# Equim-chan/Mortal

Measured on AMD Instinct MI355X. Metric: env steps/sec (65536 parallel tables per GPU), higher is better.
Workload: dtype u8/i32 state, f32 obs

## Files before the change

### mortal_amd/csrc/mj_capi.hip

```cpp
#include <hip/hip_runtime.h>

#include <algorithm>
#include <cmath>
#include <cstdio>
#include <cstring>
#include <optional>
#include <string>
#include <vector>

#include "../../include/mortal_amd.h"
#include "mj_step.hip"
#include "mj_replay.hip"
#include "mj_encode.hip"
#include "mj_sp.hip"

static_assert(sizeof(MjAlgoQuery) == 72, "MjAlgoQuery layout");
__global__ __launch_bounds__(64) void mj_k_algo_query(const MjAlgoQuery* q, int n, MjAlgoResult* out) {
    const int i = blockIdx.x * 64 + threadIdx.x;
    if (i >= n) return;
    const MjAlgoQuery Q = q[i];
    MjAlgoResult R = {0, 0, 0, 0, 0, 0, 0, 0};
    Hand h = {0, 0};
    for (int t = 0; t < 34; t++)
        for (int c = 0; c < (int)Q.tehai[t] && c < 4; c++) h.inc(t);
// ... 975 lines not shown
                    sp_[8], sp_[0], sp_[1], sp_[2], sp_[3], sp_[4], sp_[9], sp_[5], sp_[10], sp_[7]);
            for (int k = 11; k < 32; k++) fprintf(stderr, " %llu", sp_[k]);
            fprintf(stderr, "\n");
        }
    }
#endif
    if (!P) return fail("null pool");
    HIP_OK(hipStreamSynchronize((hipStream_t)stream));
    unsigned long long tmp[8];
    HIP_OK(hipMemcpy(tmp, P->counters, sizeof tmp, hipMemcpyDeviceToHost));
    for (int i = 0; i < 8; i++) out[i] = tmp[i];
    out[5] = P->cycles;
    int f = 0;
    HIP_OK(hipMemcpy(&f, P->enc_flag, sizeof f, hipMemcpyDeviceToHost));
    out[6] = (unsigned long long)f;
    if (P->sp.err) {
        unsigned long long e2[SP_ERR_WORDS];
        HIP_OK(hipMemcpy(e2, P->sp.err, sizeof e2, hipMemcpyDeviceToHost));
        out[6] += e2[SP_ERR_OVERFLOW];
        out[7] = e2[SP_ERR_ROWS];
        const unsigned long long* pass = e2 + SP_ERR_PASS;
        if (P->knobs.sp_prof)
            fprintf(stderr, "[sp prof] rows %llu setup %llu expand %llu evalL0 %llu evalL>0 %llu encode %llu states %llu (wall_clock64 ticks, 100 MHz) | "
                    "expand passes: probes %llu lists+V %llu td-probes %llu layout %llu inserts %llu; items %llu expanded %llu edges %llu l0-entries %llu; level-0 probe %llu scoring %llu; workgroup lifetimes: sum %llu max %llu queue pops %llu hash resets %llu; eval wavefront time %llu; shader clock %.0f MHz (s_memtime cycles %llu over the lifetimes)\n",
                    e2[SP_ERR_ROWS], e2[SP_ERR_T_SETUP], e2[SP_ERR_T_EXPAND], e2[SP_ERR_T_EVAL0], e2[SP_ERR_T_EVAL], e2[SP_ERR_T_WRITE], e2[SP_ERR_STATES],
                    pass[0], pass[1], pass[2], pass[3], pass[4], pass[5], pass[6], e2[SP_ERR_EDGES], e2[SP_ERR_L0_ITEMS],
                    e2[SP_ERR_T_L0_PROBE], e2[SP_ERR_T_L0_SCORE], e2[SP_ERR_WG_LIFE], e2[SP_ERR_WG_LIFE_MAX], e2[SP_ERR_T_POP], e2[SP_ERR_T_RESET],
                    e2[SP_ERR_T_EVAL_WAVE], e2[SP_ERR_WG_LIFE] ? 100.0 * (double)e2[SP_ERR_WG_CLOCK] / (double)e2[SP_ERR_WG_LIFE] : 0.0,
                    e2[SP_ERR_WG_CLOCK]);
    }
    return 0;
}

int mj_sp_phase_ticks(MjPool* P, uint64_t out[8], void* stream) {
    if (!P) return fail("null pool");
    for (int i = 0; i < 8; i++) out[i] = 0;
    if (!P->sp.err) return 0;
    HIP_OK(hipStreamSynchronize((hipStream_t)stream));
    unsigned long long e2[8];
    HIP_OK(hipMemcpy(e2, P->sp.err, sizeof e2, hipMemcpyDeviceToHost));
    for (int i = 0; i < 8; i++) out[i] = e2[i];
    return 0;
}

int mj_pool_set_sp_schedule(MjPool* P, int mode, int max_rows, int wide_grid, int min_level1, int min_level2) {
    if (!P) return fail("null pool");
    if (P->sp.work && mode != 0 && mode >= -1 && P->sp.spare == 0) return fail("mj_pool_set_sp_schedule: the work areas are allocated (call it before the first obs-v4 mj_encode)");
    if (mode >= -1) P->sp_wide_mode = mode > 0 ? 1 : mode;
    if (max_rows > 0) P->sp_wide_max_rows = max_rows;
    if (wide_grid > 0) P->sp_wide_grid = std::min(wide_grid, 256);
    if (min_level1 > 0) P->sp_promo_min[1] = min_level1;
    if (min_level2 > 0) P->sp_promo_min[2] = min_level2;
    P->sp_sched_set = true;
    return 0;
}

int mj_sp_schedule_stats(MjPool* P, uint64_t out[4], void* stream) {
    if (!P) return fail("null pool");
    for (int i = 0; i < 4; i++) out[i] = 0;
    if (!P->sp.err) return 0;
    HIP_OK(hipStreamSynchronize((hipStream_t)stream));
    unsigned long long e2[SP_ERR_WORDS];
    HIP_OK(hipMemcpy(e2, P->sp.err, sizeof e2, hipMemcpyDeviceToHost));
    out[0] = P->sp_hybrid_launches;
    out[1] = e2[SP_ERR_PROMOTED];
    out[2] = e2[SP_ERR_SWEPT];
// ... 47 lines not shown
```

### mortal_amd/csrc/mj_sp.hip

```cpp
#include <hip/hip_runtime.h>

#include <type_traits>

#include "mj_rules.h"
#include "mj_sptab.h"


#ifndef SP_THREADS
#define SP_THREADS 256
#endif
#define SP_CAP 16384
#define SP_T 17
#define SP_MAX_CAND 14
#ifndef SP_NS
#define SP_NS 16
#endif
#ifndef SP_SORT_MIN
#define SP_SORT_MIN 8
#endif
#ifndef SP_ITEM_CAP
#define SP_ITEM_CAP 64
#endif
#ifndef SP_WPS
#define SP_WPS 4
#endif
#define SP_WGS (4 * SP_WPS * 64 / SP_THREADS)

#ifndef SP_CC_N
#define SP_CC_N 2048
#endif
#ifndef SP_TAIL_BATCH
#define SP_TAIL_BATCH 4
#endif
#define SP_Q_TAIL 32
#define SP_Q_PROMO_DONE 96
#define SP_PROMO_LEVELS 2
#define SP_Q_PROMO_ALLOC(p) (128 + 64 * (p))
#define SP_Q_PROMO_HEAD(p) (160 + 64 * (p))
#define SP_Q_PROMO_ENT 256
#ifndef SP_PROMO_CAP
#define SP_PROMO_CAP 512
#endif
#define SP_Q_WORDS (SP_Q_PROMO_ENT + SP_PROMO_CAP)
#ifndef SP_WIDE_THREADS
#define SP_WIDE_THREADS 1024
#endif
#define SP_POOL (SP_CAP * 32)
#define SP_ITEMS (SP_CAP * 4)
#define SP_L0_MAX 17
#define SP_EL_SLOT(v) ((v) & (SP_CAP - 1))
#define SP_EL_IDX(v) ((v) >> 14)
struct alignas(128) SpNode {
    float val[SP_T][3];
    u8 pad_[52];
};
static_assert(sizeof(SpNode) == 256 && offsetof(SpNode, val) == 0, "SpNode layout");
struct alignas(16) SpHdr {
    u32 child_off;
    unsigned short n_ch;
    u8 sumreq, n_ent;
    u64 l0cnt2;
};
static_assert(sizeof(SpHdr) == 16 && offsetof(SpHdr, n_ch) == 4 && offsetof(SpHdr, sumreq) == 6 && offsetof(SpHdr, l0cnt2) == 8,
              "the evaluation reads the header as one or two u64");
struct SpKeys {
    u64 k0, k1, k2, k3;
    u64 dk;
};
#define SP_ENT_SLOT(e) ((e) & 0x3FFFu)
#define SP_ENT_KEY(e) (((e) >> 14) & 511u)
#define SP_ENT_LAST (1u << 23)
#define SP_ENT_COUNT(e) (((e) >> 24) & 7u)
#define SP_ENT_INVALID (1u << 27)
struct alignas(16) SpF4 { float x, y, z, w; };
#define SP_HANDOFF_WORDS 1024
struct alignas(128) SpWork {
    u64 tag[SP_CAP];
    SpNode node[SP_CAP];
    SpKeys keys[SP_CAP];
    SpHdr hdr[SP_CAP];
    u32 list[SP_CAP];
    u32 elist[SP_CAP];
    u32 pool[SP_POOL];
    u32 items[SP_ITEMS];
    SpF4 l0sc[SP_ITEMS];
    u32 epoch;
    u32 pad_[31];
    alignas(16) u32 handoff[SP_HANDOFF_WORDS];
#ifdef MJ_EMU
    u32 idx_of[SP_CAP];
#endif
};
static_assert(offsetof(SpWork, node) % 128 == 0 && sizeof(SpWork) % 128 == 0, "nodes on line boundaries");

#define SP_NT_ROWS 124
#define SP_NT_STRIDE (SP_T + 3)
__constant__ const float* c_sp_nt;
static inline void sp_not_tsumo_build(float* out ) {
    for (int n_left = 0; n_left < SP_NT_ROWS; n_left++)
        for (int q = 0; q < SP_NT_ROWS; q++) {
            float* r = out + ((size_t)n_left * SP_NT_ROWS + q) * SP_NT_STRIDE;
            const bool row_on = q <= 122 && q < n_left + 1;
            const int lim = n_left - q;
            float cur = row_on ? 1.f : 0.f;
            for (int j = 0; j < SP_NT_STRIDE; j++) r[j] = 0.f;
            r[0] = cur;
            for (int j = 0; j < SP_T - 1; j++) {
                cur = (row_on && j < lim) ? cur * (float)(n_left - q - j) / (float)(n_left - j) : 0.f;
                r[j + 1] = cur;
            }
        }
}

struct SpParams {
    const TableOne* snap;
    const uint32_t* rows;
    int n_rows;
    MjTablesDev tables;
    float* obs;
    SpWork* work;
    int* queue;
    const uint32_t* order;
    unsigned long long* prof;
// ... 68 lines not shown
};
MJD void sp_discard(SpState& s, int tile) {
    s.h.dec(deaka(tile));
    if (is_aka(tile)) s.akas &= ~(1u << (tile - T_5MR));
}
MJD void sp_deal(SpState& s, int tile) {
    s.w.dec(deaka(tile));
    s.h.inc(deaka(tile));
    if (is_aka(tile)) {
        s.akas &= ~(8u << (tile - T_5MR));
        s.akas |= 1u << (tile - T_5MR);
    }
}
MJD void sp_key(const SpState& s, u64 k[4]) {
    k[0] = s.h.mp;
    k[1] = s.h.sz | ((u64)(s.akas & 7) << 48);
    k[2] = s.w.mp;
    k[3] = s.w.sz | ((u64)((s.akas >> 3) & 7) << 48);
}

struct alignas(16) SpCtx {
    Melds melds;
    int len_div3, bakaze, jikaze, is_menzen, num_doras_in_fuuro, n_dora, calc_double_riichi, calc_haitei,
        prefer_riichi, T, n_left;
    int dora_ind[5];
    float tsumo_prob[4][SP_T];
    int lvl_begin[5], lvl_end[5];
    int n_list;
    int n_pool;
    int n_items;
    int overflow;
    unsigned long long* prof;
    unsigned long long pt[8];
    unsigned long long* cc;
    unsigned cc_epoch;
    unsigned tag_epoch;
    int n_cand;
    int cand_tile[SP_MAX_CAND], cand_slot[SP_MAX_CAND], cand_down[SP_MAX_CAND], cand_nreq[SP_MAX_CAND];
    u64 cand_req[SP_MAX_CAND];
    u64 spec_req[2][34];
    u64 row7x[2];
    signed char colcand[36];
    int order[SP_MAX_CAND];
    float cand_tp0[SP_MAX_CAND], cand_wp0[SP_MAX_CAND], cand_ev0[SP_MAX_CAND];
};

#if defined(__HIP_DEVICE_COMPILE__)
#define SP_ASSUME_LDS(p) __builtin_assume(__builtin_amdgcn_is_shared((const void*)(p)))
#else
#define SP_ASSUME_LDS(p) ((void)0)
#endif
#ifdef MJ_EMU
#define SP_HBM
#else
#define SP_HBM __attribute__((address_space(1)))
#endif

#if defined(__HIP_DEVICE_COMPILE__) && !defined(MJ_EMU)
template <class Tp> __device__ __forceinline__ Tp* sp_uniform(Tp* p) {
    const unsigned long long v = (unsigned long long)p;
    const unsigned lo = __builtin_amdgcn_readfirstlane((unsigned)v), hi = __builtin_amdgcn_readfirstlane((unsigned)(v >> 32));
    return (Tp*)(((unsigned long long)hi << 32) | lo);
}
#else
template <class Tp> MJD Tp* sp_uniform(Tp* p) { return p; }
#endif
template <class Tv, class Bp> __device__ __forceinline__ Tv sp_ld(Bp base, u32 byte_off) {
// ... 28 lines not shown
#ifdef MJ_EMU
    *reinterpret_cast<SpF3*>(reinterpret_cast<char*>(base) + byte_off) = SpF3{x, y, z};
#else
    SP_HBM SpF3* p = reinterpret_cast<SP_HBM SpF3*>(reinterpret_cast<SP_HBM char*>(base) + (unsigned long long)byte_off);
    p->x = x; p->y = y; p->z = z;
#endif
}
MJD int sp_f2i(float v) {
#if defined(MJ_EMU)
    return v != v ? 0 : v >= 2147483648.f ? 2147483647 : v <= -2147483648.f ? (-2147483647 - 1) : (int)v;
#else
    return (int)v;
#endif
}

MJD u64 sp_dk_add(u64 dk, int draw_tile, int discard_tile) {
    u32 d0 = (u32)dk & 63, d1 = (u32)(dk >> 6) & 63, d2 = (u32)(dk >> 12) & 63;
    u32 x0 = (u32)(dk >> 18) & 63, x1 = (u32)(dk >> 24) & 63, x2 = (u32)(dk >> 30) & 63, x3 = (u32)(dk >> 36) & 63;
    if (draw_tile >= 0) {
        u32 x = (u32)draw_tile + 1, t;
        t = max(d0, x); x = min(d0, x); d0 = t;
        t = max(d1, x); x = min(d1, x); d1 = t;
        d2 = max(d2, x);
    }
    if (discard_tile >= 0) {
        u32 x = (u32)discard_tile + 1, t;
        t = max(x0, x); x = min(x0, x); x0 = t;
        t = max(x1, x); x = min(x1, x); x1 = t;
        t = max(x2, x); x = min(x2, x); x2 = t;
        x3 = max(x3, x);
    }
    return (u64)(d0 | (d1 << 6) | (d2 << 12) | (x0 << 18) | (x1 << 24)) | ((u64)(x2 | (x3 << 6)) << 30);
}
MJD u32 sp_dk_pos(u64 dk) {
    u32 h = (u32)dk * 0x9E3779B1u ^ ((u32)(dk >> 32) + 0x7F4A7C15u) * 0x85EBCA77u;
    h ^= h >> 15;
    return (h * 0x2C1B3C6Du) >> 18;
}
static_assert(SP_CAP == 1 << 14, "sp_dk_pos returns 14 bits");
#define SP_EPOCH_MAX 0x1FFFFFu
#ifndef SP_EPOCH_WRAP
#define SP_EPOCH_WRAP SP_EPOCH_MAX
#endif
#define SP_TAG(dk, ep) ((dk) | ((u64)(ep) << 42) | (1ull << 63))
MJD bool sp_tag_free(u64 t, u32 ep) { return (u32)((t >> 42) & SP_EPOCH_MAX) != ep; }

#ifndef SP_OPAQUE_TID
#define SP_OPAQUE_TID 2
#endif
#if defined(MJ_EMU)
#define SP_OPQ(level, v) (v)
#else
__device__ __forceinline__ int sp_opaque_v(int v) { asm volatile("" : "+v"(v)); return v; }
#define SP_OPQ(level, v) ((SP_OPAQUE_TID) >= (level) ? sp_opaque_v(v) : (v))
#endif
#if defined(MJ_EMU) || !defined(SP_OPAQUE_PTR)
#define SP_OPQ_PTR(level, p) (p)
#else
template <typename Tp> __device__ __forceinline__ Tp* sp_opaque_s(Tp* p) { asm volatile("" : "+s"(p)); return p; }
#define SP_OPQ_PTR(level, p) ((SP_OPAQUE_PTR) >= (level) ? sp_opaque_s(p) : (p))
#endif
#ifndef SP_ATTR_EXPAND
#define SP_ATTR_EXPAND __forceinline__
#endif
#ifndef SP_ATTR_L0P
#define SP_ATTR_L0P __noinline__
#endif
#ifndef SP_ATTR_L0S
#define SP_ATTR_L0S __noinline__
#endif
#ifndef SP_ATTR_EVAL
#define SP_ATTR_EVAL __noinline__
// ... 1 lines not shown
#ifndef SP_ATTR_EVAL0
#define SP_ATTR_EVAL0 __noinline__
#endif

template <class TagP>
MJD u64 sp_claim_tag(TagP tagp, u64 h, u64 seen) {
    u64 expected = seen;
    __hip_atomic_compare_exchange_strong(tagp, &expected, h, __ATOMIC_RELAXED, __ATOMIC_RELAXED, __HIP_MEMORY_SCOPE_AGENT);
    return expected == seen ? 0ull : expected;
}
MJD SpState sp_apply(SpState s, int tile, int dt) {
    if (tile >= 0) sp_deal(s, tile);
    if (dt >= 0) sp_discard(s, dt);
    return s;
}
template <class WP>
__device__ __forceinline__ void sp_new_state(WP W, SpCtx* X, u32 slot, u64 dk, const SpState& st) {
    const int idx = atomicAdd(&X->n_list, 1);
    if (idx < SP_CAP) {
        u64 k[4];
        sp_key(st, k);
        W->list[idx] = slot;
        auto& e = W->keys[idx];
        e.k0 = k[0]; e.k1 = k[1]; e.k2 = k[2]; e.k3 = k[3]; e.dk = dk;
#ifdef MJ_EMU
        W->idx_of[slot] = (u32)idx;
#endif
    } else {
        X->overflow = 1;
    }
}
#ifdef MJ_EMU
template <class WP>
inline void sp_emu_check_hit(WP W, SpCtx* X, u32 slot, const SpState& st) {
    u64 k[4];
    sp_key(st, k);
    const auto& e = W->keys[W->idx_of[slot]];
    if (e.k0 != k[0] || e.k1 != k[1] || e.k2 != k[2] || e.k3 != k[3]) X->overflow = 1;
}
#endif
template <class WP>
__device__ __forceinline__ int sp_insert(WP W, SpCtx* X, u64 dk, const SpState& base, int tile, int dt) {
    const u32 ep = X->tag_epoch;
    const u64 tag = SP_TAG(dk, ep);
    u32 pos = sp_dk_pos(dk);
    for (int probe = 0; probe < SP_CAP; probe++) {
        u64 old = W->tag[pos];
        if (sp_tag_free(old, ep)) old = sp_claim_tag(&W->tag[pos], tag, old);
        if (old == 0ull) {
            sp_new_state(W, X, pos, dk, sp_apply(base, tile, dt));
            return (int)pos;
        }
        if (old == tag) {
#ifdef MJ_EMU
            sp_emu_check_hit(W, X, pos, sp_apply(base, tile, dt));
#endif
            return (int)pos;
        }
        pos = (pos + 1) & (SP_CAP - 1);
    }
    X->overflow = 1;
    return -1;
}
template <class NodeT>
MJD SpState sp_state_of(const NodeT& n) {
    SpState s;
    s.h.mp = n.k0;
    s.h.sz = n.k1 & 0xFFFFFFFFFFFFull;
    s.w.mp = n.k2;
    s.w.sz = n.k3 & 0xFFFFFFFFFFFFull;
    s.akas = (u32)((n.k1 >> 48) & 7) | ((u32)((n.k3 >> 48) & 7) << 3);
    return s;
}

__device__ bool sp_get_score(const MjTablesDev& T, const SpCtx* X, const SpState& s, int win_tile, float scores[4]) {
    AgariIn in;
    in.tehai = s.h;
    {
        const Melds& xm = X->melds;
        in.m.chis = xm.chis; in.m.pons = xm.pons; in.m.minkans = xm.minkans; in.m.ankans = xm.ankans;
        in.m.n_chis = xm.n_chis; in.m.n_pons = xm.n_pons; in.m.n_minkans = xm.n_minkans; in.m.n_ankans = xm.n_ankans;
    }
    in.is_menzen = X->is_menzen != 0;
    in.bakaze = X->bakaze;
    in.jikaze = X->jikaze;
    in.winning_tile = deaka(win_tile);
    in.is_ron = false;
    const bool is_oya = X->jikaze == T_E;
    const int additional = X->is_menzen ? (X->prefer_riichi ? 2 : 1) : 0;
    int num_doras = 0;
// ... 248 lines not shown
            const bool aka = sp_aka_in_wall(S, t);
            cnt += (!aka || S.w.get(t) >= 2) + aka;
            sumreq += S.w.get(t);
        }
        u64 cnt2 = 0;
        if (cnt > SP_L0_MAX) { X->overflow = 1; cnt = SP_L0_MAX; }
        const int base = atomicAdd(&X->n_items, cnt);
        int e = 0;
        for (u64 rest = req; rest; rest &= rest - 1) {
            const int t = __ffsll((long long)rest) - 1;
            const bool aka = sp_aka_in_wall(S, t);
            const int wc = S.w.get(t);
            for (int variant = 0; variant < 2; variant++) {
                if (variant == 0 ? (aka && wc < 2) : !aka) continue;
                if (e < cnt) {
                    if (base + e < SP_ITEMS) Wg->items[base + e] = (u32)(first + s) | ((u32)e << 14) | ((u32)t << 19) | ((u32)variant << 25);
                    else X->overflow = 1;
                    cnt2 |= (u64)(((!aka ? wc : variant == 0 ? wc - 1 : 1) - 1) & 3) << (2 * e);
                }
                e++;
            }
        }
        (void)slot;
        SP_HBM SpHdr& hd = Wg->hdr[first + s];
        hd.child_off = (u32)min(base, SP_ITEMS - 1);
        hd.n_ch = (unsigned short)cnt;
        hd.sumreq = (u8)(sumreq & 0xFF);
        hd.n_ent = (u8)cnt;
        hd.l0cnt2 = cnt2;
    }
    mj_team_sync<SP_NT>();
}

__device__ SP_ATTR_EXPAND void sp_expand_chunk(SpWork* W, SpCtx* X, SpChunk* C, int first, int n, int L) {
    SP_ASSUME_LDS(X);
    SP_ASSUME_LDS(C);
    SP_HBM SpWork* const Wg = (SP_HBM SpWork*)SP_OPQ_PTR(2, W);
    const SpTabG TG = sp_tab_g(*SP_OPQ_PTR(1, &c_sp_tab));
    const int tid = SP_OPQ(1, (int)(threadIdx.x & (SP_NT - 1)));
    const int ld3 = X->len_div3;
    const u32 tag_ep = X->tag_epoch;
    const bool prof = X->prof != nullptr;
    long long tq0 = prof ? wall_clock64() : 0, tq1 = 0;
    long long acc_list = 0, acc_keep = 0, acc_layout = 0, acc_ins = 0;
    int n_items_total = 0, n_edges_total = 0;
    sp_chunk_probe(Wg, X, C, TG, first, n, L);
    if (prof) tq1 = wall_clock64();
    const long long t_probe = tq1 - tq0;

    const int nt_lane = tid < n ? (int)C->n_tiles[tid] : 0;
    const int pre_in = (int)sp_wave_scan_incl((u32)nt_lane), pre_ex = pre_in - nt_lane;
    const int total_items = sp_lane_get(pre_in, SP_NT - 1);
    const int n_sub = (total_items + SP_ITEM_CAP - 1) / SP_ITEM_CAP, target = n_sub > 1 ? (total_items + n_sub - 1) / n_sub : SP_ITEM_CAP;
    for (int sb = 0; sb < n;) {
        long long tp0 = prof ? wall_clock64() : 0, tp1 = 0, tp2 = 0, tp3 = 0, tp4 = 0;
        const int base = sp_lane_get(pre_ex, sb);
        const bool stop = tid > sb && tid < n && (pre_in - base > SP_ITEM_CAP || pre_ex - base >= target);
        const u64 stop_m = __ballot(stop);
        const int se = stop_m ? __ffsll((long long)stop_m) - 1 : n;
        const int n_items = sp_lane_get(pre_ex, se) - base;
        const int my_first = pre_ex - base;
        if (tid >= sb && tid < se) {
            const int s = tid;
            int it = my_first;
            for (u64 rest = C->req[s]; rest; rest &= rest - 1) C->item[it++] = (unsigned short)(s | ((__ffsll((long long)rest) - 1) << SP_SB));
            if (it == my_first) {
// ... 59 lines not shown
                const int e_first = (int)((pv & 0xFFFFu) - (u32)my_ent);
                C->eoff[tid] = (unsigned short)e_first;
                {
                    int r = 0;
                    for (u64 rest = kept; rest; rest &= rest - 1, r++) {
                        const u32 d = (u32)(__ffsll((long long)rest) - 1);
                        const u32 w = (u32)tid | (d << 6) | ((rest & (rest - 1)) == 0ull ? 1u << 13 : 0u);
                        if (e_first + r < SP_EINFO_CAP) C->einfo[e_first + r] = w;
                        if (nvar == 2 && e_first + nkeep + r < SP_EINFO_CAP) C->einfo[e_first + nkeep + r] = w | (1u << 12);
                    }
                }
                if (tid == s_last) {
                    const u32 tot = upto - base;
                    int total = (int)(tot & 0xFFFFu);
                    const int sumreq = (int)((tot >> 16) & 0xFFu), n_ent = (int)(tot >> 24);
                    int child_base = atomicAdd(&X->n_pool, total);
                    if (child_base + total > SP_POOL) { X->overflow = 1; child_base = SP_POOL; total = 0; }
                    C->child_base[my_s] = child_base;
                    SP_HBM SpHdr& hd = Wg->hdr[first + my_s];
                    hd.child_off = (u32)min(child_base, SP_POOL - 1);
                    hd.n_ch = (unsigned short)total;
                    hd.sumreq = (u8)(sumreq & 0xFF);
                    hd.n_ent = (u8)min(n_ent, 255);
                }
            }
            if (tid == 0) C->eoff[n_items] = (unsigned short)n_entries;
        }
        mj_team_sync<SP_NT>();
        if (prof) tp3 = wall_clock64();
        struct Ent {
            bool on;
            int s, it, local, rank, nk, tile, dt, count;
            u64 dk;
            u32 pos;
        };
        auto decode = [&](int e) -> Ent {
            Ent E;
            E.on = e < n_entries;
            const int ee = E.on ? e : 0;
            int lo, vidx, d;
            if (ee < SP_EINFO_CAP) {
                const u32 w = C->einfo[ee];
                lo = (int)(w & 63u);
                d = (int)((w >> 6) & 63u);
                vidx = (int)((w >> 12) & 1u);
                E.local = ee - (int)C->eoff[lo];
                E.nk = 2;
                E.rank = (w >> 13) & 1u ? 1 : 0;
            } else {
                lo = 0;
                int hi = n_items;
                while (hi - lo > 1) {
                    const int mid = (lo + hi) >> 1;
                    if ((int)C->eoff[mid] <= ee) lo = mid; else hi = mid;
                }
                E.local = ee - (int)C->eoff[lo];
                const u64 bits = C->kept[lo];
                E.nk = __popcll(bits);
                vidx = E.local >= E.nk ? 1 : 0;
                E.rank = E.local - vidx * E.nk;
                u64 mrest = bits;
                for (int r = E.rank; r > 0; r--) mrest &= mrest - 1;
                d = __ffsll((long long)mrest) - 1;
            }
            E.it = lo;
            E.s = C->item[lo] & (SP_NS - 1);
            const int t = C->item[lo] >> SP_SB;
            const SpState Sx = sp_chunk_state(C, E.s);
            const int cnt = Sx.w.get(t);
            const bool aka = sp_aka_in_wall(Sx, t);
            const bool red = aka && (vidx == 1 || cnt < 2);
            E.count = !aka ? cnt : red ? 1 : cnt - 1;
            E.tile = red ? akaize(t) : t;
            const u32 akas1 = red ? (Sx.akas | (1u << (E.tile - T_5MR))) : Sx.akas;
            const int c = Sx.h.get(d & 63);
            int dt = d;
            if (d == T_5M && (akas1 & 1) && c == 1) dt = T_5MR;
            else if (d == T_5P && (akas1 & 2) && c == 1) dt = T_5PR;
            else if (d == T_5S && (akas1 & 4) && c == 1) dt = T_5SR;
            E.dt = dt;
            E.dk = sp_dk_add(C->dk[E.s], E.tile, dt);
            E.pos = sp_dk_pos(E.dk);
            return E;
        };
        auto finish = [&](const Ent& E, u64 first_old, int known) -> int {
            const u64 tag = SP_TAG(E.dk, tag_ep);
            const SpState Sx = sp_chunk_state(C, E.s);
            u32 pos = E.pos;
            u64 old = first_old;
            int cs = known;
            bool fresh = false;
#ifdef MJ_EMU
            if (known >= 0 && Wg->tag[known] != tag) X->overflow = 1;
#endif
            for (int probe = 0; cs < 0 && probe < SP_CAP; probe++) {
                if (old == 0ull) {
                    fresh = true;
                    cs = (int)pos;
                    break;
                }
                if (old == tag) {
#ifdef MJ_EMU
                    sp_emu_check_hit(Wg, X, pos, sp_apply(Sx, E.tile, E.dt));
#endif
                    cs = (int)pos;
                    break;
                }
                pos = (pos + 1) & (SP_CAP - 1);
                old = Wg->tag[pos];
                if (sp_tag_free(old, tag_ep)) old = sp_claim_tag(&Wg->tag[pos], tag, old);
            }
            if (cs < 0) X->overflow = 1;
            if (fresh) sp_new_state(Wg, X, (u32)cs, E.dk, sp_apply(Sx, E.tile, E.dt));
            const int pos_out = C->child_base[E.s] + (int)C->coff[E.it] + E.local;
            const u32 ent = (cs < 0 ? SP_ENT_INVALID : (u32)cs) | ((u32)sp_discard_key(E.dt) << 14) | (E.rank == E.nk - 1 ? SP_ENT_LAST : 0u) |
                            ((u32)E.count << 24);
            if (pos_out < SP_POOL) Wg->pool[pos_out] = ent;
            return cs;
        };
#if SP_CC_N > 0
        unsigned long long* const cc = X->cc;
        SP_ASSUME_LDS(cc);
#else
        unsigned long long* const cc = nullptr;
#endif
        const u64 cc_ep = (u64)X->cc_epoch << 42;
        auto cc_look = [&](const Ent& E) -> int {
            if (!cc || !E.on) return -1;
            const u64 v = cc[E.pos & (SP_CC_N - 1)];
            return (v >> 14) == (cc_ep | E.dk) ? (int)(v & 0x3FFFu) : -1;
        };
        auto cc_put = [&](const Ent& E, int cs) {
            if (cc && cs >= 0) cc[E.pos & (SP_CC_N - 1)] = ((cc_ep | E.dk) << 14) | (u64)(u32)cs;
        };
        for (int e0 = 0; e0 < n_entries; e0 += 2 * SP_NT) {
            const bool two = e0 + SP_NT < n_entries;
            const Ent A = decode(e0 + tid);
            Ent B = A;
            B.on = false;
            if (two) B = decode(e0 + SP_NT + tid);
            u64 oa = 1ull, ob = 1ull;
            const int ka = cc_look(A), kb = cc_look(B);
            if (A.on && ka < 0) oa = Wg->tag[A.pos];
            if (B.on && kb < 0) ob = Wg->tag[B.pos];
            if (A.on && ka < 0 && sp_tag_free(oa, tag_ep)) oa = sp_claim_tag(&Wg->tag[A.pos], SP_TAG(A.dk, tag_ep), oa);
            if (B.on && kb < 0 && sp_tag_free(ob, tag_ep)) ob = sp_claim_tag(&Wg->tag[B.pos], SP_TAG(B.dk, tag_ep), ob);
            if (A.on) {
                const int cs = finish(A, oa, ka);
                if (ka < 0) cc_put(A, cs);
            }
            if (B.on) {
                const int cs = finish(B, ob, kb);
                if (kb < 0) cc_put(B, cs);
            }
        }
        mj_team_sync<SP_NT>();
        if (prof) {
            tp4 = wall_clock64();
            acc_list += tp1 - tp0;
            acc_keep += tp2 - tp1;
            acc_layout += tp3 - tp2;
            acc_ins += tp4 - tp3;
            n_items_total += n_items;
            n_edges_total += n_entries;
        }
        sb = se;
    }
    if (prof && tid == 0) {
        atomicAdd(&X->pt[0], (unsigned long long)t_probe);
        atomicAdd(&X->pt[1], (unsigned long long)acc_list);
        atomicAdd(&X->pt[2], (unsigned long long)acc_keep);
        atomicAdd(&X->pt[3], (unsigned long long)acc_layout);
        atomicAdd(&X->pt[4], (unsigned long long)acc_ins);
        atomicAdd(&X->pt[5], (unsigned long long)n_items_total);
        atomicAdd(&X->pt[6], (unsigned long long)n);
    }
}

#define SP_EVAL_LDS_FLOATS(NT) (((NT) / 64) * 1408)
// ... 275 lines not shown
                }
            });
        }
        mj_team_sync<64>();

        if (done) {
            sp_st3(nodeB, SP_EL_SLOT(s0) * (u32)sizeof(SpNode) + val_ln, acc_t, acc_w, acc_e);
            s0 = s1; s1 = s2; s2 = s3; s3 = s4;
            h0 = h1; h1 = h2; h2 = h3;
            m_raw = m_nxt; m_nxt = m_n2;
#pragma unroll
            for (int q = 0; q < SP_EV_ENT; q++) nent[q] = nent2[q];
            c0 = 0;
            my_m = m_raw != 0.f ? m_raw : 1.f;
            my_r = sp_rcp_refined(my_m);
            acc_t = acc_w = acc_e = 0.f;
            i += stride;
            has = i < end;
        }
#pragma unroll
        for (int q = 0; q < SP_EV_ENT; q++) {
            ent[q] = up[q];
            entn[q] = upn[q];
            v[q] = vn[q];
        }
    }
}

template <int NT>
__device__ __forceinline__ void sp_sort_level(SpWork* W, int* hist , int b, int e) {
    SP_HBM SpWork* const Wg = (SP_HBM SpWork*)W;
    const int tid = threadIdx.x;
    if (e - b <= SP_SORT_MIN) {
        for (int i = b + tid; i < e; i += NT) Wg->elist[i] = Wg->list[i] | ((u32)i << 14);
        __syncthreads();
        return;
    }
    if (tid < 64) hist[tid] = 0;
    __syncthreads();
    auto cost_key = [&](int i) {
        const SP_HBM SpHdr& hd = Wg->hdr[i];
        return 63 - min(((int)hd.n_ch + 4 * (int)hd.n_ent) >> 1, 63);
    };
    u32 my_slot[4];
    int my_key[4];
#pragma unroll
    for (int q = 0; q < 4; q++) {
        const int i = b + tid + q * NT;
        my_slot[q] = i < e ? (Wg->list[i] | ((u32)i << 14)) : 0u;
        my_key[q] = i < e ? cost_key(i) : 0;
        if (i < e) atomicAdd(&hist[my_key[q]], 1);
    }
    for (int i = b + tid + 4 * NT; i < e; i += NT) atomicAdd(&hist[cost_key(i)], 1);
    __syncthreads();
    if (tid < 64) {
        const int c = hist[tid];
        hist[tid] = (int)sp_wave_scan_incl((u32)c) - c;
    }
    __syncthreads();
#pragma unroll
    for (int q = 0; q < 4; q++) {
        const int i = b + tid + q * NT;
        if (i < e) Wg->elist[b + atomicAdd(&hist[my_key[q]], 1)] = my_slot[q];
    }
    for (int i = b + tid + 4 * NT; i < e; i += NT) Wg->elist[b + atomicAdd(&hist[cost_key(i)], 1)] = Wg->list[i] | ((u32)i << 14);
    __syncthreads();
}

MJD int f32_total_cmp(float a, float b) {
    int x = __float_as_int(a), y = __float_as_int(b);
    x ^= (int)((unsigned)(x >> 31) >> 1);
    y ^= (int)((unsigned)(y >> 31) >> 1);
    return (x > y) - (x < y);
}

#define SP_N_CLASS 8
MJD int sp_row_class(const TableOne* snap, uint32_t desc) {
    LaneT<TableOne> L;
    L.B = const_cast<TableOne*>(snap + ROW_TABLE(desc));
    L.l = 0;
    L.T = nullptr;
    const int p = ROW_SEAT(desc);
    const u32 cans = F1(cans, p);
    const bool cd = (cans & CAN_DISCARD) != 0;
    const int tiles_left = F(tiles_left);
    int sh = F1(shanten, p), tsumos_left;
    if (cd) {
        if (sh > 0 && F1(has_next_shanten, p)) sh -= 1;
        tsumos_left = tiles_left / 4;
    } else {
        const int target = (F1(cans_target, p) + 4 - p) & 3;
        tsumos_left = max(tiles_left - (4 - target), 0) / 4;
    }
    if (tiles_left < 4 || sh > 3 || tsumos_left < max(sh, 1)) return 7;
    if (sh <= 1) return 6;
    if (sh == 2) return cd ? 4 : 5;
    if (!cd) return 2;
    const int n_cand = __popcll(F1(has_next_shanten, p) ? F1(next_shanten, p) : F1(keep_shanten, p));
// ... 426 lines not shown
#define SP_DRAIN_STORES() asm volatile("s_waitcnt vmcnt(0)" ::: "memory")
#define SP_RELEASE_AGENT() do { __builtin_amdgcn_fence(__ATOMIC_RELEASE, "agent"); asm volatile("s_waitcnt vmcnt(0)" ::: "memory"); } while (0)
#define SP_ACQUIRE_AGENT() __builtin_amdgcn_fence(__ATOMIC_ACQUIRE, "agent")
#define SP_SPIN_PAUSE() __builtin_amdgcn_s_sleep(32)
#else
#define SP_DRAIN_STORES() ((void)0)
#define SP_RELEASE_AGENT() ((void)0)
#define SP_ACQUIRE_AGENT() ((void)0)
#define SP_SPIN_PAUSE() ((void)0)
#endif

#ifdef SP_ROWDUMP
#define SP_DUMP(P) ((P).rowdump != nullptr)
#else
#define SP_DUMP(P) false
#endif
template <int NT>
struct SpLds {
    union Teams {
        TableOne st;
        SpChunk wchunk[NT / SP_NT];
        float ev[SP_EVAL_LDS_FLOATS(NT)];
        SpWaveArea wave[NT / 64];
    };
};

template <int NT, bool WIDE, bool PROMO>
__device__ __forceinline__ void sp_kernel_body(SpParams P) {
    __shared__ SpCtx X;
    __shared__ int s_row, s_k;
    __shared__ unsigned long long s_stat[SP_ERR_STATS];
    if (threadIdx.x < SP_ERR_STATS) s_stat[threadIdx.x] = 0ull;
    __shared__ typename SpLds<NT>::Teams s_tm;
#if SP_CC_N > 0
    __shared__ unsigned long long s_cc[SP_CC_N];
    for (int i = threadIdx.x; i < SP_CC_N; i += NT) s_cc[i] = 0ull;
    unsigned n_graph_rows = 0;
#endif
    SpWork* W = WIDE ? P.work + P.n_narrow + P.promo_cap + blockIdx.x : P.work + blockIdx.x;
    SpWork* const W_own = W;
    const int tid_wg = threadIdx.x, tid = tid_wg;

    unsigned tag_epoch = W->epoch;
    unsigned own_epoch = tag_epoch;
    bool main_done = false, drained = false;

    const long long t_wg_in = SP_DUMP(P) ? wall_clock64() : 0;
    const long long t_wg0 = P.prof ? wall_clock64() : 0;
#ifndef MJ_EMU
    const long long c_wg0 = P.prof ? clock64() : 0;
#endif
    long long t_pop = 0, t_reset = 0;
    const int n_heavy = P.n_rows - P.queue[1 + 7];
    bool wave_mode = false;
    for (;;) {
        const int tid = SP_OPQ(2, tid_wg);
        const long long t_a = P.prof ? wall_clock64() : 0;
        int row, lv_first = 0;
        SpRowInfo R;
        long long t_0, t_1, t_2, t_3, t_4;
        bool promoted = false;
        if constexpr (WIDE) {
            if (tid == 0) {
                int got = 0;
                const int cap = P.promo_cap / SP_PROMO_LEVELS;
                long long t_idle = 0;
                for (;;) {
                    for (int q = 0; q < SP_PROMO_LEVELS && !got; q++) {
                        int* const ents = P.queue + SP_Q_PROMO_ENT + q * (SP_PROMO_CAP / SP_PROMO_LEVELS);
                        int* const head = P.queue + SP_Q_PROMO_HEAD(q) + (P.sweep ? 1 : 0);
                        for (;;) {
// ... 54 lines not shown
                row = H->row;
                lv_first = H->next_lv;
                __syncthreads();
                tag_epoch = X.tag_epoch;
            } else {
                W = W_own;
                tag_epoch = own_epoch;
                row = (int)P.order[-s_row - 1];
            }
            t_1 = t_2 = t_3 = t_4 = t_0;
        } else {
            if (tid == 0) s_row = atomicAdd(P.queue, 1);
            __syncthreads();
            if (s_row >= n_heavy) { wave_mode = n_heavy < P.n_rows; break; }
            row = (int)P.order[s_row];
            if (P.prof) t_pop += wall_clock64() - t_a;
            t_0 = wall_clock64();
            t_1 = t_2 = t_3 = t_4 = t_0;
        }
        float* out = P.obs + (size_t)row * (1012 * 34);
        if (!promoted) {
            R = sp_row_front<false, NT>(P.rows, P.snap, W, X, &s_tm.st, tid, row, out, P.prof);
            if (!R.ok) continue;
        }
        const int cur_shanten = R.cur_shanten, n_cand = R.n_cand, T = R.T;
        const bool with_probs = R.with_probs, can_discard = R.can_discard;
        const SpState root = R.root;
        if (!promoted) {
            t_1 = wall_clock64();
            t_2 = t_3 = t_4 = t_1;
        }
        bool parked = false;
        if (with_probs) {
#if SP_CC_N > 0
            n_graph_rows++;
            if ((n_graph_rows & 255u) == 0u) {
                n_graph_rows++;
                for (int i = tid; i < SP_CC_N; i += NT) s_cc[i] = 0ull;
            }
            if (tid == 0) {
                X.cc = s_cc;
                X.cc_epoch = n_graph_rows & 255u;
            }
#else
            if (tid == 0) X.cc = nullptr;
#endif
            if (promoted) {
                if (tid == 0) {
                    X.prof = P.prof;
                    for (int k = 0; k < 8; k++) X.pt[k] = 0ull;
                }
                __syncthreads();
            } else {
                if (tag_epoch >= SP_EPOCH_WRAP) {
                    for (int i = tid; i < SP_CAP; i += NT) W->tag[i] = 0ull;
                    tag_epoch = 0;
                    __syncthreads();
                }
                tag_epoch++;
                if (tid == 0) X.tag_epoch = tag_epoch;
                __syncthreads();
                if (tid < n_cand) {
                    const int c = tid;
                    SpState s = root;
                    if (can_discard) sp_discard(s, X.cand_tile[c]);
                    X.cand_slot[c] = sp_insert(W, &X, sp_dk_add(0ull, -1, can_discard ? X.cand_tile[c] : -1), s, -1, -1);
                }
                __syncthreads();
                if (tid == 0) {
                    X.lvl_begin[cur_shanten] = 0;
                    X.lvl_end[cur_shanten] = X.n_list;
                }
                __syncthreads();
            }
            for (int lv = promoted ? lv_first : cur_shanten; lv >= 1; lv--) {
                const int b = X.lvl_begin[lv], e = X.lvl_end[lv];
                if constexpr (PROMO) {
                    if (P.promo_cap > 0 && lv < cur_shanten && e - b >= P.promo_min[lv] && !X.overflow) {
                        const int pq = e - b >= 2 * P.promo_min[lv] ? 0 : 1;
                        if (tid == 0) s_k = atomicAdd(P.queue + SP_Q_PROMO_ALLOC(pq), 1);
                        __syncthreads();
                        const int k = s_k;
                        if (k < P.promo_cap / SP_PROMO_LEVELS) {
                            {
                                const u32* sx = reinterpret_cast<const u32*>(&X);
                                SP_HBM u32* dst = (SP_HBM u32*)W->handoff;
                                for (int i = tid; i < (int)(sizeof(SpCtx) / 4); i += NT) dst[i] = sx[i];
                                if (tid == 0) {
                                    SpHandoff* H = reinterpret_cast<SpHandoff*>(W->handoff);
                                    H->R = R;
                                    H->row = row;
                                    H->next_lv = lv;
                                    W->epoch = tag_epoch;
                                    if (SP_DUMP(P)) P.rowdump[(size_t)row * 12 + 8] = (uint32_t)t_0, P.rowdump[(size_t)row * 12 + 9] = (uint32_t)wall_clock64();
                                }
                            }
                            SP_DRAIN_STORES();
                            __syncthreads();
                            if (tid == 0) {
                                SP_RELEASE_AGENT();
                                __hip_atomic_store(P.queue + SP_Q_PROMO_ENT + pq * (SP_PROMO_CAP / SP_PROMO_LEVELS) + k, (int)(W - P.work) + 1, __ATOMIC_RELAXED,
                                                   __HIP_MEMORY_SCOPE_AGENT);
                            }
                            W = P.work + gridDim.x + pq * (P.promo_cap / SP_PROMO_LEVELS) + k;
                            tag_epoch = W->epoch;
                            parked = true;
                            break;
                        }
                    }
                }
                const int ns = min(SP_NS, max(1, (e - b + NT / SP_NT - 1) / (NT / SP_NT)));
                for (int c0 = b + ns * (tid / SP_NT); c0 < e; c0 += ns * (NT / SP_NT))
                    sp_expand_chunk(W, &X, &s_tm.wchunk[tid / SP_NT], c0, min(ns, e - c0), lv);
                __syncthreads();
                if (tid == 0) {
                    X.lvl_begin[lv - 1] = e;
                    X.lvl_end[lv - 1] = min(X.n_list, SP_CAP);
                }
                __syncthreads();
            }
            t_2 = wall_clock64();
            if (!parked)
            for (int lv = 0; lv <= cur_shanten; lv++) {
                const int b = X.lvl_begin[lv], e = X.lvl_end[lv];
                if (lv == 0) {
                    if (tid == 0) X.n_items = 0;
                    __syncthreads();
                    const int ns = min(SP_NS, max(1, (e - b + NT / SP_NT - 1) / (NT / SP_NT)));
                    for (int c0 = b + ns * (tid / SP_NT); c0 < e; c0 += ns * (NT / SP_NT))
                        sp_l0_probe_chunk(W, &X, &s_tm.wchunk[tid / SP_NT], c0, min(ns, e - c0));
                    __syncthreads();
                    const long long t_2a = wall_clock64();
                    const int n_items = min(X.n_items, SP_ITEMS);
                    if ((tid & ~63) < n_items) sp_l0_score_all(c_mj_tables, W, &X, n_items, tid, NT);
                    __syncthreads();
                    if (P.prof && tid == 0) {
                        X.pt[7] += (unsigned long long)(t_2a - t_2);
                        s_stat[SP_ERR_T_L0_SCORE] += (unsigned long long)(wall_clock64() - t_2a);
                    }
                }
                sp_sort_level<NT>(W, reinterpret_cast<int*>(s_tm.ev), b, e);
                {
                    const int off = min(cur_shanten - lv, T - 1), TW = T - off;
                    const int wl = tid & 63, tw = wl / TW, ln = wl - tw * TW;
                    float* wl_lds = s_tm.ev + (tid >> 6) * SP_EVW_WAVE_FLOATS;
                    const long long t_ev0 = P.prof ? wall_clock64() : 0;
// ... 130 lines not shown
```

Measured before the change: 4.170 million.

## Replace LDS child cache with LDS two-choice cuckoo-style set owning node slots

For narrow, non-promoted workgroups, the LDS lookaside cache of global hash slots becomes an authoritative two-bucket set in LDS. Tags are claimed there, and states that fit get dedicated node slots placed ahead of the global table, which falls back to the HBM tag probe only when both buckets are full. Slot fields widen from 14 to 15 bits to address the extra nodes. This is meant to cut HBM tag reads and atomic claims during expansion, at the cost of a larger SpWork node array and more LDS atomics, plus a set reset on every epoch wrap.

```diff
diff --git a/mortal_amd/csrc/mj_capi.hip b/mortal_amd/csrc/mj_capi.hip
--- a/mortal_amd/csrc/mj_capi.hip
+++ b/mortal_amd/csrc/mj_capi.hip
@@ -1031,6 +1031,10 @@
     return 0;
 }
 
+#ifdef MJ_EMU
+void mj_emu_sp_placed(uint64_t out[2]) { out[0] = g_sp_emu_placed[0]; out[1] = g_sp_emu_placed[1]; }
+#endif
+
 int mj_sp_phase_ticks(MjPool* P, uint64_t out[8], void* stream) {
     if (!P) return fail("null pool");
     for (int i = 0; i < 8; i++) out[i] = 0;
diff --git a/mortal_amd/csrc/mj_sp.hip b/mortal_amd/csrc/mj_sp.hip
--- a/mortal_amd/csrc/mj_sp.hip
+++ b/mortal_amd/csrc/mj_sp.hip
@@ -26,9 +26,12 @@
 #endif
 #define SP_WGS (4 * SP_WPS * 64 / SP_THREADS)
 
-#ifndef SP_CC_N
-#define SP_CC_N 2048
-#endif
+#ifndef SP_SET_BUCKETS
+#define SP_SET_BUCKETS 1024
+#endif
+#define SP_SET_SLOTS (2 * SP_SET_BUCKETS)
+#define SP_NODES (SP_CAP + SP_SET_SLOTS)
+static_assert((SP_SET_BUCKETS & (SP_SET_BUCKETS - 1)) == 0 && SP_SET_BUCKETS >= 1 && SP_NODES <= (1 << 15), "slots are 15-bit fields");
 #ifndef SP_TAIL_BATCH
 #define SP_TAIL_BATCH 4
 #endif
@@ -48,8 +51,8 @@
 #define SP_POOL (SP_CAP * 32)
 #define SP_ITEMS (SP_CAP * 4)
 #define SP_L0_MAX 17
-#define SP_EL_SLOT(v) ((v) & (SP_CAP - 1))
-#define SP_EL_IDX(v) ((v) >> 14)
+#define SP_EL_SLOT(v) ((v) & 0x7FFFu)
+#define SP_EL_IDX(v) ((v) >> 15)
 struct alignas(128) SpNode {
     float val[SP_T][3];
     u8 pad_[52];
@@ -67,16 +70,16 @@
     u64 k0, k1, k2, k3;
     u64 dk;
 };
-#define SP_ENT_SLOT(e) ((e) & 0x3FFFu)
-#define SP_ENT_KEY(e) (((e) >> 14) & 511u)
-#define SP_ENT_LAST (1u << 23)
-#define SP_ENT_COUNT(e) (((e) >> 24) & 7u)
-#define SP_ENT_INVALID (1u << 27)
+#define SP_ENT_SLOT(e) ((e) & 0x7FFFu)
+#define SP_ENT_KEY(e) (((e) >> 15) & 511u)
+#define SP_ENT_LAST (1u << 24)
+#define SP_ENT_COUNT(e) (((e) >> 25) & 7u)
+#define SP_ENT_INVALID (1u << 28)
 struct alignas(16) SpF4 { float x, y, z, w; };
 #define SP_HANDOFF_WORDS 1024
 struct alignas(128) SpWork {
     u64 tag[SP_CAP];
-    SpNode node[SP_CAP];
+    SpNode node[SP_NODES];
     SpKeys keys[SP_CAP];
     SpHdr hdr[SP_CAP];
     u32 list[SP_CAP];
@@ -88,7 +91,7 @@
     u32 pad_[31];
     alignas(16) u32 handoff[SP_HANDOFF_WORDS];
 #ifdef MJ_EMU
-    u32 idx_of[SP_CAP];
+    u32 idx_of[SP_NODES];
 #endif
 };
 static_assert(offsetof(SpWork, node) % 128 == 0 && sizeof(SpWork) % 128 == 0, "nodes on line boundaries");
@@ -223,7 +226,7 @@
     int overflow;
     unsigned long long* prof;
     unsigned long long pt[8];
-    unsigned long long* cc;
+    u64* set;
     unsigned cc_epoch;
     unsigned tag_epoch;
     int n_cand;
@@ -318,12 +321,17 @@
     }
     return (u64)(d0 | (d1 << 6) | (d2 << 12) | (x0 << 18) | (x1 << 24)) | ((u64)(x2 | (x3 << 6)) << 30);
 }
-MJD u32 sp_dk_pos(u64 dk) {
+MJD u32 sp_dk_hash(u64 dk) {
     u32 h = (u32)dk * 0x9E3779B1u ^ ((u32)(dk >> 32) + 0x7F4A7C15u) * 0x85EBCA77u;
     h ^= h >> 15;
-    return (h * 0x2C1B3C6Du) >> 18;
-}
-static_assert(SP_CAP == 1 << 14, "sp_dk_pos returns 14 bits");
+    return h * 0x2C1B3C6Du;
+}
+MJD u32 sp_hash_pos(u32 h) { return h >> 18; }
+MJD u32 sp_dk_pos(u64 dk) { return sp_hash_pos(sp_dk_hash(dk)); }
+static_assert(SP_CAP == 1 << 14, "sp_hash_pos returns 14 bits");
+MJD u32 sp_hash_b1(u32 h) { return (h >> 8) & (SP_SET_BUCKETS - 1); }
+MJD u32 sp_hash_b2(u32 h) { return (h >> 18) & (SP_SET_BUCKETS - 1); }
+static_assert(SP_SET_BUCKETS <= 1024, "two disjoint 10-bit fields of the hash");
 #define SP_EPOCH_MAX 0x1FFFFFu
 #ifndef SP_EPOCH_WRAP
 #define SP_EPOCH_WRAP SP_EPOCH_MAX
@@ -391,30 +399,69 @@
 }
 #ifdef MJ_EMU
 template <class WP>
-inline void sp_emu_check_hit(WP W, SpCtx* X, u32 slot, const SpState& st) {
+inline void sp_emu_check_hit(WP W, SpCtx* X, u32 slot, u64 dk, const SpState& st) {
     u64 k[4];
     sp_key(st, k);
-    const auto& e = W->keys[W->idx_of[slot]];
-    if (e.k0 != k[0] || e.k1 != k[1] || e.k2 != k[2] || e.k3 != k[3]) X->overflow = 1;
-}
-#endif
-template <class WP>
+    const u32 idx = W->idx_of[slot];
+    if (idx >= (u32)SP_CAP) return;
+    const auto& e = W->keys[idx];
+    if (e.dk == dk && (e.k0 != k[0] || e.k1 != k[1] || e.k2 != k[2] || e.k3 != k[3])) X->overflow = 1;
+}
+inline unsigned long long g_sp_emu_placed[2];
+#endif
+__device__ __forceinline__ int sp_set_find_or_claim(u64* set, u32 h, u64 tag, u32 ep) {
+    struct alignas(16) Bucket { u64 w[2]; };
+    const u32 b[2] = {sp_hash_b1(h), sp_hash_b2(h)};
+    const Bucket B0 = reinterpret_cast<const Bucket*>(set)[b[0]], B1 = reinterpret_cast<const Bucket*>(set)[b[1]];
+    const u64 w[4] = {B0.w[0], B0.w[1], B1.w[0], B1.w[1]};
+#pragma unroll
+    for (int i = 0; i < 4; i++)
+        if (w[i] == tag) return (int)(2 * b[i >> 1] + (i & 1));
+#pragma unroll
+    for (int i = 0; i < 4; i++) {
+        if (!sp_tag_free(w[i], ep)) continue;
+        const u32 slot = 2 * b[i >> 1] + (i & 1);
+        const u64 old = sp_claim_tag(&set[slot], tag, w[i]);
+        if (old == 0ull) return (int)slot | (1 << 16);
+        if (old == tag) return (int)slot;
+    }
+    return -1;
+}
+template <bool LDS_SET, class WP>
 __device__ __forceinline__ int sp_insert(WP W, SpCtx* X, u64 dk, const SpState& base, int tile, int dt) {
     const u32 ep = X->tag_epoch;
     const u64 tag = SP_TAG(dk, ep);
-    u32 pos = sp_dk_pos(dk);
+    const u32 h = sp_dk_hash(dk);
+    constexpr u32 HB = LDS_SET ? SP_SET_SLOTS : 0;
+    if constexpr (LDS_SET) {
+        u64* const set = X->set;
+        SP_ASSUME_LDS(set);
+        const int r = sp_set_find_or_claim(set, h, tag, ep);
+        if (r >= 0) {
+            if (r >> 16) sp_new_state(W, X, (u32)(r & 0xFFFF), dk, sp_apply(base, tile, dt));
+#ifdef MJ_EMU
+            if (r >> 16) g_sp_emu_placed[0]++;
+            else sp_emu_check_hit(W, X, (u32)r, dk, sp_apply(base, tile, dt));
+#endif
+            return r & 0xFFFF;
+        }
+    }
+    u32 pos = sp_hash_pos(h);
     for (int probe = 0; probe < SP_CAP; probe++) {
         u64 old = W->tag[pos];
         if (sp_tag_free(old, ep)) old = sp_claim_tag(&W->tag[pos], tag, old);
         if (old == 0ull) {
-            sp_new_state(W, X, pos, dk, sp_apply(base, tile, dt));
-            return (int)pos;
+            sp_new_state(W, X, HB + pos, dk, sp_apply(base, tile, dt));
+#ifdef MJ_EMU
+            g_sp_emu_placed[1]++;
+#endif
+            return (int)(HB + pos);
         }
         if (old == tag) {
 #ifdef MJ_EMU
-            sp_emu_check_hit(W, X, pos, sp_apply(base, tile, dt));
-#endif
-            return (int)pos;
+            sp_emu_check_hit(W, X, HB + pos, dk, sp_apply(base, tile, dt));
+#endif
+            return (int)(HB + pos);
         }
         pos = (pos + 1) & (SP_CAP - 1);
     }
@@ -729,6 +776,7 @@
     mj_team_sync<SP_NT>();
 }
 
+template <bool LDS_SET>
 __device__ SP_ATTR_EXPAND void sp_expand_chunk(SpWork* W, SpCtx* X, SpChunk* C, int first, int n, int L) {
     SP_ASSUME_LDS(X);
     SP_ASSUME_LDS(C);
@@ -854,7 +902,7 @@
             bool on;
             int s, it, local, rank, nk, tile, dt, count;
             u64 dk;
-            u32 pos;
+            u32 h;
         };
         auto decode = [&](int e) -> Ent {
             Ent E;
@@ -902,30 +950,36 @@
             else if (d == T_5S && (akas1 & 4) && c == 1) dt = T_5SR;
             E.dt = dt;
             E.dk = sp_dk_add(C->dk[E.s], E.tile, dt);
-            E.pos = sp_dk_pos(E.dk);
+            E.h = sp_dk_hash(E.dk);
             return E;
         };
+        constexpr u32 HB = LDS_SET ? SP_SET_SLOTS : 0;
         auto finish = [&](const Ent& E, u64 first_old, int known) -> int {
             const u64 tag = SP_TAG(E.dk, tag_ep);
             const SpState Sx = sp_chunk_state(C, E.s);
-            u32 pos = E.pos;
+            u32 pos = sp_hash_pos(E.h);
             u64 old = first_old;
-            int cs = known;
-            bool fresh = false;
+            int cs = known >= 0 ? (known & 0xFFFF) : -1;
+            bool fresh = known >= 0 && (known >> 16) != 0;
 #ifdef MJ_EMU
-            if (known >= 0 && Wg->tag[known] != tag) X->overflow = 1;
+            if (LDS_SET && known >= 0 && !fresh) sp_emu_check_hit(Wg, X, (u32)cs, E.dk, sp_apply(Sx, E.tile, E.dt));
+            if (!LDS_SET && known >= 0 && Wg->tag[known] != tag) X->overflow = 1;
+            if (fresh) g_sp_emu_placed[0]++;
 #endif
             for (int probe = 0; cs < 0 && probe < SP_CAP; probe++) {
                 if (old == 0ull) {
                     fresh = true;
-                    cs = (int)pos;
+                    cs = (int)(HB + pos);
+#ifdef MJ_EMU
+                    g_sp_emu_placed[1]++;
+#endif
                     break;
                 }
                 if (old == tag) {
 #ifdef MJ_EMU
-                    sp_emu_check_hit(Wg, X, pos, sp_apply(Sx, E.tile, E.dt));
-#endif
-                    cs = (int)pos;
+                    sp_emu_check_hit(Wg, X, HB + pos, E.dk, sp_apply(Sx, E.tile, E.dt));
+#endif
+                    cs = (int)(HB + pos);
                     break;
                 }
                 pos = (pos + 1) & (SP_CAP - 1);
@@ -935,25 +989,25 @@
             if (cs < 0) X->overflow = 1;
             if (fresh) sp_new_state(Wg, X, (u32)cs, E.dk, sp_apply(Sx, E.tile, E.dt));
             const int pos_out = C->child_base[E.s] + (int)C->coff[E.it] + E.local;
-            const u32 ent = (cs < 0 ? SP_ENT_INVALID : (u32)cs) | ((u32)sp_discard_key(E.dt) << 14) | (E.rank == E.nk - 1 ? SP_ENT_LAST : 0u) |
-                            ((u32)E.count << 24);
+            const u32 ent = (cs < 0 ? SP_ENT_INVALID : (u32)cs) | ((u32)sp_discard_key(E.dt) << 15) | (E.rank == E.nk - 1 ? SP_ENT_LAST : 0u) |
+                            ((u32)E.count << 25);
             if (pos_out < SP_POOL) Wg->pool[pos_out] = ent;
             return cs;
         };
-#if SP_CC_N > 0
-        unsigned long long* const cc = X->cc;
-        SP_ASSUME_LDS(cc);
-#else
-        unsigned long long* const cc = nullptr;
-#endif
+        u64* const set = X->set;
+        SP_ASSUME_LDS(set);
         const u64 cc_ep = (u64)X->cc_epoch << 42;
-        auto cc_look = [&](const Ent& E) -> int {
-            if (!cc || !E.on) return -1;
-            const u64 v = cc[E.pos & (SP_CC_N - 1)];
-            return (v >> 14) == (cc_ep | E.dk) ? (int)(v & 0x3FFFu) : -1;
+        auto look = [&](const Ent& E) -> int {
+            if (!E.on) return -1;
+            if constexpr (LDS_SET) {
+                return sp_set_find_or_claim(set, E.h, SP_TAG(E.dk, tag_ep), tag_ep);
+            } else {
+                const u64 v = set[sp_hash_pos(E.h) & (SP_SET_SLOTS - 1)];
+                return (v >> 14) == (cc_ep | E.dk) ? (int)(v & 0x3FFFu) : -1;
+            }
         };
         auto cc_put = [&](const Ent& E, int cs) {
-            if (cc && cs >= 0) cc[E.pos & (SP_CC_N - 1)] = ((cc_ep | E.dk) << 14) | (u64)(u32)cs;
+            if (!LDS_SET && cs >= 0) set[sp_hash_pos(E.h) & (SP_SET_SLOTS - 1)] = ((cc_ep | E.dk) << 14) | (u64)(u32)cs;
         };
         for (int e0 = 0; e0 < n_entries; e0 += 2 * SP_NT) {
             const bool two = e0 + SP_NT < n_entries;
@@ -962,11 +1016,12 @@
             B.on = false;
             if (two) B = decode(e0 + SP_NT + tid);
             u64 oa = 1ull, ob = 1ull;
-            const int ka = cc_look(A), kb = cc_look(B);
-            if (A.on && ka < 0) oa = Wg->tag[A.pos];
-            if (B.on && kb < 0) ob = Wg->tag[B.pos];
-            if (A.on && ka < 0 && sp_tag_free(oa, tag_ep)) oa = sp_claim_tag(&Wg->tag[A.pos], SP_TAG(A.dk, tag_ep), oa);
-            if (B.on && kb < 0 && sp_tag_free(ob, tag_ep)) ob = sp_claim_tag(&Wg->tag[B.pos], SP_TAG(B.dk, tag_ep), ob);
+            const int ka = look(A), kb = look(B);
+            const u32 pa = sp_hash_pos(A.h), pb = sp_hash_pos(B.h);
+            if (A.on && ka < 0) oa = Wg->tag[pa];
+            if (B.on && kb < 0) ob = Wg->tag[pb];
+            if (A.on && ka < 0 && sp_tag_free(oa, tag_ep)) oa = sp_claim_tag(&Wg->tag[pa], SP_TAG(A.dk, tag_ep), oa);
+            if (B.on && kb < 0 && sp_tag_free(ob, tag_ep)) ob = sp_claim_tag(&Wg->tag[pb], SP_TAG(B.dk, tag_ep), ob);
             if (A.on) {
                 const int cs = finish(A, oa, ka);
                 if (ka < 0) cc_put(A, cs);
@@ -1308,7 +1363,7 @@
     SP_HBM SpWork* const Wg = (SP_HBM SpWork*)W;
     const int tid = threadIdx.x;
     if (e - b <= SP_SORT_MIN) {
-        for (int i = b + tid; i < e; i += NT) Wg->elist[i] = Wg->list[i] | ((u32)i << 14);
+        for (int i = b + tid; i < e; i += NT) Wg->elist[i] = Wg->list[i] | ((u32)i << 15);
         __syncthreads();
         return;
     }
@@ -1323,7 +1378,7 @@
 #pragma unroll
     for (int q = 0; q < 4; q++) {
         const int i = b + tid + q * NT;
-        my_slot[q] = i < e ? (Wg->list[i] | ((u32)i << 14)) : 0u;
+        my_slot[q] = i < e ? (Wg->list[i] | ((u32)i << 15)) : 0u;
         my_key[q] = i < e ? cost_key(i) : 0;
         if (i < e) atomicAdd(&hist[my_key[q]], 1);
     }
@@ -1339,7 +1394,7 @@
         const int i = b + tid + q * NT;
         if (i < e) Wg->elist[b + atomicAdd(&hist[my_key[q]], 1)] = my_slot[q];
     }
-    for (int i = b + tid + 4 * NT; i < e; i += NT) Wg->elist[b + atomicAdd(&hist[cost_key(i)], 1)] = Wg->list[i] | ((u32)i << 14);
+    for (int i = b + tid + 4 * NT; i < e; i += NT) Wg->elist[b + atomicAdd(&hist[cost_key(i)], 1)] = Wg->list[i] | ((u32)i << 15);
     __syncthreads();
 }
 
@@ -1832,11 +1887,10 @@
     __shared__ unsigned long long s_stat[SP_ERR_STATS];
     if (threadIdx.x < SP_ERR_STATS) s_stat[threadIdx.x] = 0ull;
     __shared__ typename SpLds<NT>::Teams s_tm;
-#if SP_CC_N > 0
-    __shared__ unsigned long long s_cc[SP_CC_N];
-    for (int i = threadIdx.x; i < SP_CC_N; i += NT) s_cc[i] = 0ull;
+    constexpr bool LDS_SET = !WIDE && !PROMO;
+    __shared__ __attribute__((aligned(16))) u64 s_set[SP_SET_SLOTS];
+    for (int i = threadIdx.x; i < SP_SET_SLOTS; i += NT) s_set[i] = 0ull;
     unsigned n_graph_rows = 0;
-#endif
     SpWork* W = WIDE ? P.work + P.n_narrow + P.promo_cap + blockIdx.x : P.work + blockIdx.x;
     SpWork* const W_own = W;
     const int tid_wg = threadIdx.x, tid = tid_wg;
@@ -1957,19 +2011,17 @@
         }
         bool parked = false;
         if (with_probs) {
-#if SP_CC_N > 0
-            n_graph_rows++;
-            if ((n_graph_rows & 255u) == 0u) {
+            if constexpr (!LDS_SET) {
                 n_graph_rows++;
-                for (int i = tid; i < SP_CC_N; i += NT) s_cc[i] = 0ull;
+                if ((n_graph_rows & 255u) == 0u) {
+                    n_graph_rows++;
+                    for (int i = tid; i < SP_SET_SLOTS; i += NT) s_set[i] = 0ull;
+                }
             }
             if (tid == 0) {
-                X.cc = s_cc;
+                X.set = s_set;
                 X.cc_epoch = n_graph_rows & 255u;
             }
-#else
-            if (tid == 0) X.cc = nullptr;
-#endif
             if (promoted) {
                 if (tid == 0) {
                     X.prof = P.prof;
@@ -1979,6 +2031,8 @@
             } else {
                 if (tag_epoch >= SP_EPOCH_WRAP) {
                     for (int i = tid; i < SP_CAP; i += NT) W->tag[i] = 0ull;
+                    if constexpr (LDS_SET)
+                        for (int i = tid; i < SP_SET_SLOTS; i += NT) s_set[i] = 0ull;
                     tag_epoch = 0;
                     __syncthreads();
                 }
@@ -1989,7 +2043,7 @@
                     const int c = tid;
                     SpState s = root;
                     if (can_discard) sp_discard(s, X.cand_tile[c]);
-                    X.cand_slot[c] = sp_insert(W, &X, sp_dk_add(0ull, -1, can_discard ? X.cand_tile[c] : -1), s, -1, -1);
+                    X.cand_slot[c] = sp_insert<LDS_SET>(W, &X, sp_dk_add(0ull, -1, can_discard ? X.cand_tile[c] : -1), s, -1, -1);
                 }
                 __syncthreads();
                 if (tid == 0) {
@@ -2036,7 +2090,7 @@
                 }
                 const int ns = min(SP_NS, max(1, (e - b + NT / SP_NT - 1) / (NT / SP_NT)));
                 for (int c0 = b + ns * (tid / SP_NT); c0 < e; c0 += ns * (NT / SP_NT))
-                    sp_expand_chunk(W, &X, &s_tm.wchunk[tid / SP_NT], c0, min(ns, e - c0), lv);
+                    sp_expand_chunk<LDS_SET>(W, &X, &s_tm.wchunk[tid / SP_NT], c0, min(ns, e - c0), lv);
                 __syncthreads();
                 if (tid == 0) {
                     X.lvl_begin[lv - 1] = e;
```

Result: faster. 4.343 million (median of 6 runs) (+4.1%).
